# rail-berkeley/serl

Hardware: NVIDIA H100
Metric: drq_critic_grad_steps_per_sec (higher is better)
Workload: dtype f16

## Files before the change

### serl_b200/csrc/stem_pool.cu

```cuda
#include "common.cuh"
#include "conv_common.cuh"
#include "serl_b200.h"
#include "wgmma.cuh"

namespace serl {

constexpr int SP_BOX = 7 * 64 * 32;
constexpr int SP_STAGE = 4 * SP_BOX;
constexpr int SP_STAGES = 3;
constexpr int SP_OFF_A = 4 * 8192;
constexpr int SP_OFF_STG = SP_OFF_A + SP_STAGES * SP_STAGE;
constexpr int SP_OFF_SLOT = SP_OFF_STG + 8 * 1024;
constexpr int SP_OFF_BAR = SP_OFF_SLOT + 4 * 4 * 4 * 2 * 4;
constexpr int SP_SMEM = SP_OFF_BAR + 8 * (2 * SP_STAGES + 5) + 1024;
static_assert((SP_BOX % 1024) == 0 && SP_SMEM <= 232448, "stem_pool_kernel: shared memory layout");

struct StemPoolArgs {
  uint16_t* pooled; uint16_t* side; float* stats; int32_t* error;
  unsigned long long neg_mask; int N;
};

template <class F>
__global__ void __launch_bounds__(CONV_THREADS, 1)
stem_pool_kernel(const __grid_constant__ CUtensorMap xmap, const __grid_constant__ CUtensorMap wmap, const StemPoolArgs a) {
  pdl_prologue();
  extern __shared__ uint8_t smem_raw[];
  uint8_t* smem = reinterpret_cast<uint8_t*>((reinterpret_cast<uintptr_t>(smem_raw) + 1023) & ~(uintptr_t)1023);
  uint8_t* sW = smem;
  uint8_t* sA = smem + SP_OFF_A;
  float* slot = reinterpret_cast<float*>(smem + SP_OFF_SLOT);
  uint64_t* full = reinterpret_cast<uint64_t*>(smem + SP_OFF_BAR);
  uint64_t* empty = full + SP_STAGES;
  uint64_t* wbar = empty + SP_STAGES;
  uint64_t* gnbar = wbar + 1;

  const int warp = threadIdx.x >> 5, lane = threadIdx.x & 31;
  const int band = blockIdx.x & 3;
  const int img0 = blockIdx.x >> 2, img_step = gridDim.x >> 2;

  if (threadIdx.x == 0) {
    for (int s = 0; s < SP_STAGES; ++s) { tc_mbar_init(&full[s], 1); tc_mbar_init(&empty[s], 4); }
    tc_mbar_init(wbar, 1);
    for (int q = 0; q < 4; ++q) tc_mbar_init(&gnbar[q], 1);
    asm volatile("fence.mbarrier_init.release.cluster;" ::: "memory");
  }
  __syncthreads();
  cluster_sync_all();

  if (warp >= 8) {
    asm volatile("setmaxnreg.dec.sync.aligned.u32 40;" ::: "memory");
    if (warp == 8 && lane == 0) {
      asm volatile("prefetch.tensormap [%0];" ::"l"(&xmap) : "memory");
      asm volatile("prefetch.tensormap [%0];" ::"l"(&wmap) : "memory");
      tc_mbar_expect_tx(wbar, 4u * 8192u);
      for (int t = 0; t < 4; ++t) tc_tma_2d(sW + t * 8192, &wmap, t * 64, 0, wbar);
      bool ok = true;
      int pos = 0;
      for (int m = 0; ok; ++m) {
        const int n0 = img0 + 2 * m * img_step;
        if (n0 >= a.N) break;
        const int imgs = n0 + img_step < a.N ? 2 : 1;
        for (int c = 0; c < 4 && ok; ++c)
          for (int g = 0; g < imgs; ++g, ++pos) {
            const int s = pos % SP_STAGES;
            if (!(ok = tc_mbar_wait(&empty[s], ((uint32_t)(pos / SP_STAGES) & 1u) ^ 1u, a.error))) break;
            tc_mbar_expect_tx(&full[s], (uint32_t)SP_STAGE);
            for (int sx = 0; sx < 4; ++sx)
              tc_tma_4d(sA + s * SP_STAGE + sx * SP_BOX, &xmap, 0, sx, 16 * band + 4 * c, n0 + g * img_step, &full[s]);
          }
      }
    }
  } else {
    asm volatile("setmaxnreg.inc.sync.aligned.u32 232;" ::: "memory");
    const int g = warp >> 2, wl = warp & 3, tid = threadIdx.x & 127, quad = lane & 3;
    const uint32_t a_base = smem_u32(sA), w_base = smem_u32(sW);
    const int ch = 16 * wl + (lane >> 2);
    const uint32_t flip = (uint32_t)((a.neg_mask >> ch) & 1ull) * 0x8000u | (uint32_t)((a.neg_mask >> (ch + 8)) & 1ull) * 0x80000000u;
    const int next = (lane & ~3) | ((lane + 1) & 3);
    uint8_t* stg = smem + SP_OFF_STG + warp * 1024;
    const uint32_t mrow = smem_u32(stg) + (uint32_t)(((lane >> 4) * 8 + (lane & 1) * 4 + ((lane >> 1) & 3)) * 32 +
                                                     ((((lane >> 3) ^ lane) & 1) << 4));
    const int gpx = lane >> 1, gh = lane & 1;
    const uint32_t grow = (uint32_t)(gpx * 32 + ((gh ^ (gpx >> 2)) & 1) * 16);
    auto store_row = [&](uint16_t* dst, const uint32_t (&v)[8]) {
      uint32_t o[2][4];
#pragma unroll
      for (int t = 0; t < 4; ++t) {
        o[t >> 1][2 * (t & 1)] = __byte_perm(v[2 * t], v[2 * t + 1], 0x5410);
        o[t >> 1][2 * (t & 1) + 1] = __byte_perm(v[2 * t], v[2 * t + 1], 0x7632);
      }
      stsm_x4_trans(mrow, o[0]);
      stsm_x4_trans(mrow + 512, o[1]);
      __syncwarp();
#pragma unroll
      for (int e = 0; e < 2; ++e)
        *reinterpret_cast<uint4*>(dst + (size_t)(gpx + 16 * e) * 64 + 8 * gh) = *reinterpret_cast<const uint4*>(stg + grow + e * 512);
      __syncwarp();
    };
    bool ok = tc_mbar_wait(wbar, 0u, a.error);
    ok = mma_bar_and(ok);
    auto collect = [&](int m) {
      const int q = 2 * g + (m & 1);
      ok = tc_mbar_wait_cluster(&gnbar[q], (uint32_t)(m >> 1) & 1u, a.error);
      if (ok && band == 0 && lane < 2) {
        float v = 0.f;
#pragma unroll
        for (int rk = 0; rk < 4; ++rk) v += slot[((q * 4 + rk) * 4 + wl) * 2 + lane];
        atomicAdd(a.stats + (size_t)(img0 + (2 * m + g) * img_step) * 8 + wl * 2 + lane, v);
      }
    };
    float acc[128];
    uint32_t carry[8];
    float S = 0.f, SS = 0.f;
    int m = 0;
    for (;; ++m) {
      const int n = img0 + (2 * m + g) * img_step;
      if (n >= a.N) break;
      const bool pair = img0 + (2 * m + 1) * img_step < a.N;
      const bool more = img0 + (2 * m + 2) * img_step < a.N;
      uint16_t* out = a.pooled + (size_t)n * 32 * 2048 + 16 * wl;
      for (int c = 0; c < 4; ++c) {
        const int pos = 8 * m + (pair ? 2 * c + g : c), s = pos % SP_STAGES;
        if (g == 1 || (c > 0 ? pair : m > 0)) named_bar_sync(2 + g, 256);
        if (ok) ok = tc_mbar_wait(&full[s], (uint32_t)(pos / SP_STAGES) & 1u, a.error);
        if (ok) {
          const uint32_t bs = a_base + (uint32_t)(s * SP_STAGE);
          wg_fence();
#pragma unroll
          for (int r = 0; r < 4; ++r)
#pragma unroll
            for (int sx = 0; sx < 4; ++sx)
              wg_mma_h16_n256<F::kBf16>(acc, wg_desc(w_base + (uint32_t)(r * 8192)) + 2 * sx,
                                        wg_desc_sw32(bs + (uint32_t)(sx * SP_BOX + r * 2048)), (uint32_t)(r | sx));
          wg_commit();
        }
        if (g == 0 ? pair : (c < 3 || more)) named_bar_arrive(3 - g, 256);
        wg_wait<0>();
        __syncwarp();
        if (!ok) continue;
        if (lane == 0) tc_mbar_arrive(&empty[s]);

        if (c == 0) {
          if (m > 0) collect(m - 1);
          S = 0.f; SS = 0.f;
        }
#pragma unroll
        for (int j = 0; j < 32; ++j) {
          const float* d = &acc[4 * j];
          S += (d[0] + d[1]) + (d[2] + d[3]);
          SS += (d[0] * d[0] + d[1] * d[1]) + (d[2] * d[2] + d[3] * d[3]);
        }
        uint32_t v[8];
        auto pool_row = [&](int i, bool first) {
          uint32_t w0[8], w1[8];
#pragma unroll
          for (int jj = 0; jj < 8; ++jj) {
            const float* d = &acc[4 * (8 * i + jj)];
            w0[jj] = F::pack(d[0], d[2]) ^ flip;
            w1[jj] = F::pack(d[1], d[3]) ^ flip;
          }
#pragma unroll
          for (int jj = 0; jj < 8; ++jj) {
            const uint32_t nb = __shfl_sync(0xffffffffu, quad == 0 ? w0[jj < 7 ? jj + 1 : 7] : w0[jj], next);
            uint32_t x = first ? w0[jj] : F::max2(v[jj], w0[jj]);
            x = F::max2(x, w1[jj]);
            if (jj < 7 || quad != 3) x = F::max2(x, nb);
            v[jj] = x;
          }
        };
        const int p0 = 8 * band + 2 * c;
        uint32_t o[8];
        pool_row(0, true);
        if (c > 0) {
#pragma unroll
          for (int jj = 0; jj < 8; ++jj) o[jj] = F::max2(carry[jj], v[jj]);
          store_row(out + (size_t)(p0 - 1) * 2048, o);
        } else {
          store_row(a.side + ((size_t)n * 4 + band) * 2048 + 16 * wl, v);
        }
        pool_row(1, false);
#pragma unroll
        for (int jj = 0; jj < 8; ++jj) o[jj] = v[jj];
        pool_row(2, true);
#pragma unroll
        for (int jj = 0; jj < 8; ++jj) o[jj] = F::max2(o[jj], v[jj]);
        store_row(out + (size_t)p0 * 2048, o);
        pool_row(3, false);
        if (c == 3) store_row(out + (size_t)(p0 + 1) * 2048, v);
#pragma unroll
        for (int jj = 0; jj < 8; ++jj) carry[jj] = v[jj];

        if (c == 3) {
          S = warp_sum(S); SS = warp_sum(SS);
          const int q = 2 * g + (m & 1);
          if (tid == 0) tc_mbar_expect_tx(&gnbar[q], 4u * 4u * 2u * 4u);
          if (lane < 2) {
            const float* dst = slot + ((q * 4 + band) * 4 + wl) * 2 + lane;
#pragma unroll
            for (int rk = 0; rk < 4; ++rk) {
              uint32_t rdst, rbar;
              asm volatile("mapa.shared::cluster.u32 %0, %1, %2;" : "=r"(rdst) : "r"(smem_u32(dst)), "r"(rk));
              asm volatile("mapa.shared::cluster.u32 %0, %1, %2;" : "=r"(rbar) : "r"(smem_u32(&gnbar[q])), "r"(rk));
              asm volatile("st.async.shared::cluster.mbarrier::complete_tx::bytes.b32 [%0], %1, [%2];"
                           ::"r"(rdst), "r"(__float_as_uint(lane ? SS : S)), "r"(rbar) : "memory");
            }
          }
        }
      }
    }
    if (ok && m > 0) collect(m - 1);
  }
  cluster_sync_all();
}

template <class F>
static int launch_stem_pool(const serl_stem_pool_desc* d, cudaStream_t st) {
  auto kern = stem_pool_kernel<F>;
  static int clusters = 0;
  if (!clusters) {
    if (cudaFuncSetAttribute(kern, cudaFuncAttributeMaxDynamicSharedMemorySize, SP_SMEM) != cudaSuccess) return check_launch("cudaFuncSetAttribute(stem_pool)");
    int dev = 0, sms = 0, n = 0;
    cudaGetDevice(&dev);
    cudaDeviceGetAttribute(&sms, cudaDevAttrMultiProcessorCount, dev);
    cudaLaunchConfig_t cfg = {};
    cudaLaunchAttribute attr[1];
    attr[0].id = cudaLaunchAttributeClusterDimension;
    attr[0].val.clusterDim.x = 4; attr[0].val.clusterDim.y = 1; attr[0].val.clusterDim.z = 1;
    cfg.gridDim = dim3(4 * sms); cfg.blockDim = dim3(CONV_THREADS); cfg.dynamicSmemBytes = SP_SMEM;
    cfg.attrs = attr; cfg.numAttrs = 1;
    if (cudaOccupancyMaxActiveClusters(&n, kern, &cfg) != cudaSuccess) return check_launch("cudaOccupancyMaxActiveClusters(stem_pool)");
    if (n <= 0) { set_last_error("serl_stem_conv_pool_tc_h16: stem_pool_kernel (%d B shared memory) cannot be resident", SP_SMEM); return SERL_ERR_CUDA; }
    clusters = n;
  }
  TcEncodeTiledFn enc = tc_get_encode();
  if (!enc) { set_last_error("serl_stem_conv_pool_tc_h16: cuTensorMapEncodeTiled unavailable"); return SERL_ERR_CUDA; }
  const CUtensorMapDataType dt = d->fmt == SERL_FMT_FP16 ? CU_TENSOR_MAP_DATA_TYPE_FLOAT16 : CU_TENSOR_MAP_DATA_TYPE_BFLOAT16;
  CUtensorMap xmap, wmap;
  {
    const cuuint64_t gdim[4] = {16u, 67u, 67u, (cuuint64_t)d->N};
    const cuuint64_t gstr[3] = {16u * 2u, 67u * 16u * 2u, 67u * 67u * 16u * 2u};
    const cuuint32_t box[4] = {16u, 64u, 7u, 1u};
    const cuuint32_t estr[4] = {1u, 1u, 1u, 1u};
    CUresult r = enc(&xmap, dt, 4, const_cast<void*>(d->xs), gdim, gstr, box, estr, CU_TENSOR_MAP_INTERLEAVE_NONE, CU_TENSOR_MAP_SWIZZLE_32B,
                     CU_TENSOR_MAP_L2_PROMOTION_L2_256B, CU_TENSOR_MAP_FLOAT_OOB_FILL_NONE);
    if (r != CUDA_SUCCESS) { set_last_error("serl_stem_conv_pool_tc_h16: cuTensorMapEncodeTiled (input) failed (%d)", (int)r); return SERL_ERR_CUDA; }
  }
  {
    const cuuint64_t gdim[2] = {256u, 64u};
    const cuuint64_t gstr[1] = {256u * 2u};
    const cuuint32_t box[2] = {64u, 64u};
    const cuuint32_t estr[2] = {1u, 1u};
    CUresult r = enc(&wmap, dt, 2, const_cast<void*>(d->w), gdim, gstr, box, estr, CU_TENSOR_MAP_INTERLEAVE_NONE, CU_TENSOR_MAP_SWIZZLE_128B,
                     CU_TENSOR_MAP_L2_PROMOTION_L2_256B, CU_TENSOR_MAP_FLOAT_OOB_FILL_NONE);
    if (r != CUDA_SUCCESS) { set_last_error("serl_stem_conv_pool_tc_h16: cuTensorMapEncodeTiled (weights) failed (%d)", (int)r); return SERL_ERR_CUDA; }
  }
  StemPoolArgs a{};
  a.pooled = static_cast<uint16_t*>(d->pooled); a.side = static_cast<uint16_t*>(d->side); a.stats = d->stats; a.error = d->error;
  a.neg_mask = d->neg_mask; a.N = d->N;
  const int rounds = ceil_div(d->N, clusters);
  const int used = ceil_div(d->N, rounds);
  launch_k_cluster(kern, dim3(used * 4), dim3(CONV_THREADS), 4, (size_t)SP_SMEM, st, xmap, wmap, a);
  return check_launch("stem_pool_kernel");
}

}

using namespace serl;

extern "C" int serl_stem_v2_active(void) { return 1; }

extern "C" int serl_stem_conv_pool_tc_h16(const serl_stem_pool_desc* d, void* stream) {
  if (!d || !d->xs || !d->w || !d->pooled || !d->side || !d->stats || !d->error || d->N < 1) {
    set_last_error("serl_stem_conv_pool_tc_h16: invalid descriptor"); return SERL_ERR_INVALID;
  }
  return d->fmt == SERL_FMT_FP16 ? launch_stem_pool<Fp16>(d, static_cast<cudaStream_t>(stream))
                                 : launch_stem_pool<Bf16>(d, static_cast<cudaStream_t>(stream));
}
```

Measured before the change: 522.2.

## Load one input box plus edge strip via TMA and build shifted copies in smem

Instead of issuing four overlapping TMA loads (one per x-shift) for each stage, the producer loads a single 64-wide box plus an 8-wide edge strip. Warps 9-11 and lane 0 of warp 8 then construct the three shifted copies with shared-memory copies and signal the full barrier. This cuts redundant global/L2 traffic by roughly 4x per stage. In exchange it adds a new loaded barrier, extra smem copy work in low-register producer warps, and a proxy fence per stage.

```diff
diff --git a/serl_b200/csrc/stem_pool.cu b/serl_b200/csrc/stem_pool.cu
--- a/serl_b200/csrc/stem_pool.cu
+++ b/serl_b200/csrc/stem_pool.cu
@@ -6,23 +6,36 @@
 namespace serl {
 
 constexpr int SP_BOX = 7 * 64 * 32;
-constexpr int SP_STAGE = 4 * SP_BOX;
+constexpr int SP_EDGE = 7 * 8 * 32;
+constexpr int SP_OFF_EDGE = 4 * SP_BOX;
+constexpr int SP_STAGE = SP_OFF_EDGE + 2048;
 constexpr int SP_STAGES = 3;
 constexpr int SP_OFF_A = 4 * 8192;
 constexpr int SP_OFF_STG = SP_OFF_A + SP_STAGES * SP_STAGE;
 constexpr int SP_OFF_SLOT = SP_OFF_STG + 8 * 1024;
 constexpr int SP_OFF_BAR = SP_OFF_SLOT + 4 * 4 * 4 * 2 * 4;
-constexpr int SP_SMEM = SP_OFF_BAR + 8 * (2 * SP_STAGES + 5) + 1024;
-static_assert((SP_BOX % 1024) == 0 && SP_SMEM <= 232448, "stem_pool_kernel: shared memory layout");
+constexpr int SP_SMEM = SP_OFF_BAR + 8 * (3 * SP_STAGES + 5) + 1024;
+static_assert((SP_BOX % 1024) == 0 && (SP_STAGE % 1024) == 0 && SP_EDGE <= SP_STAGE - SP_OFF_EDGE && SP_SMEM <= 232448,
+              "stem_pool_kernel: shared memory layout");
 
 struct StemPoolArgs {
   uint16_t* pooled; uint16_t* side; float* stats; int32_t* error;
   unsigned long long neg_mask; int N;
 };
 
+__device__ __forceinline__ uint4 lds128(uint32_t addr) {
+  uint4 v;
+  asm volatile("ld.shared.v4.b32 {%0, %1, %2, %3}, [%4];" : "=r"(v.x), "=r"(v.y), "=r"(v.z), "=r"(v.w) : "r"(addr) : "memory");
+  return v;
+}
+__device__ __forceinline__ void sts128(uint32_t addr, const uint4& v) {
+  asm volatile("st.shared.v4.b32 [%0], {%1, %2, %3, %4};" ::"r"(addr), "r"(v.x), "r"(v.y), "r"(v.z), "r"(v.w) : "memory");
+}
+
 template <class F>
 __global__ void __launch_bounds__(CONV_THREADS, 1)
-stem_pool_kernel(const __grid_constant__ CUtensorMap xmap, const __grid_constant__ CUtensorMap wmap, const StemPoolArgs a) {
+stem_pool_kernel(const __grid_constant__ CUtensorMap xmap, const __grid_constant__ CUtensorMap emap,
+                 const __grid_constant__ CUtensorMap wmap, const StemPoolArgs a) {
   pdl_prologue();
   extern __shared__ uint8_t smem_raw[];
   uint8_t* smem = reinterpret_cast<uint8_t*>((reinterpret_cast<uintptr_t>(smem_raw) + 1023) & ~(uintptr_t)1023);
@@ -31,7 +44,8 @@
   float* slot = reinterpret_cast<float*>(smem + SP_OFF_SLOT);
   uint64_t* full = reinterpret_cast<uint64_t*>(smem + SP_OFF_BAR);
   uint64_t* empty = full + SP_STAGES;
-  uint64_t* wbar = empty + SP_STAGES;
+  uint64_t* loaded = empty + SP_STAGES;
+  uint64_t* wbar = loaded + SP_STAGES;
   uint64_t* gnbar = wbar + 1;
 
   const int warp = threadIdx.x >> 5, lane = threadIdx.x & 31;
@@ -39,7 +53,7 @@
   const int img0 = blockIdx.x >> 2, img_step = gridDim.x >> 2;
 
   if (threadIdx.x == 0) {
-    for (int s = 0; s < SP_STAGES; ++s) { tc_mbar_init(&full[s], 1); tc_mbar_init(&empty[s], 4); }
+    for (int s = 0; s < SP_STAGES; ++s) { tc_mbar_init(&full[s], 3); tc_mbar_init(&empty[s], 4); tc_mbar_init(&loaded[s], 1); }
     tc_mbar_init(wbar, 1);
     for (int q = 0; q < 4; ++q) tc_mbar_init(&gnbar[q], 1);
     asm volatile("fence.mbarrier_init.release.cluster;" ::: "memory");
@@ -51,9 +65,18 @@
     asm volatile("setmaxnreg.dec.sync.aligned.u32 40;" ::: "memory");
     if (warp == 8 && lane == 0) {
       asm volatile("prefetch.tensormap [%0];" ::"l"(&xmap) : "memory");
+      asm volatile("prefetch.tensormap [%0];" ::"l"(&emap) : "memory");
       asm volatile("prefetch.tensormap [%0];" ::"l"(&wmap) : "memory");
       tc_mbar_expect_tx(wbar, 4u * 8192u);
       for (int t = 0; t < 4; ++t) tc_tma_2d(sW + t * 8192, &wmap, t * 64, 0, wbar);
+    }
+    if (warp > 8 || lane == 0) {
+      const int sx = warp - 8, xl = lane >> 1, h = lane & 1, xs = xl + sx;
+      const uint32_t src = (uint32_t)(xs * 32 + ((h ^ (xs >> 2)) & 1) * 16);
+      const uint32_t dst = (uint32_t)(sx * SP_BOX + xl * 32 + ((h ^ (xl >> 2)) & 1) * 16);
+      const int e = xs - 16;
+      const uint32_t src3 = e < 0 ? 1536u + src : (uint32_t)(SP_OFF_EDGE + e * 32 + ((h ^ (e >> 2)) & 1) * 16);
+      const uint32_t step3 = e < 0 ? 2048u : 256u;
       bool ok = true;
       int pos = 0;
       for (int m = 0; ok; ++m) {
@@ -63,10 +86,29 @@
         for (int c = 0; c < 4 && ok; ++c)
           for (int g = 0; g < imgs; ++g, ++pos) {
             const int s = pos % SP_STAGES;
-            if (!(ok = tc_mbar_wait(&empty[s], ((uint32_t)(pos / SP_STAGES) & 1u) ^ 1u, a.error))) break;
-            tc_mbar_expect_tx(&full[s], (uint32_t)SP_STAGE);
-            for (int sx = 0; sx < 4; ++sx)
-              tc_tma_4d(sA + s * SP_STAGE + sx * SP_BOX, &xmap, 0, sx, 16 * band + 4 * c, n0 + g * img_step, &full[s]);
+            const uint32_t par = (uint32_t)(pos / SP_STAGES) & 1u;
+            if (warp == 8) {
+              if (!(ok = tc_mbar_wait(&empty[s], par ^ 1u, a.error))) break;
+              tc_mbar_expect_tx(&loaded[s], (uint32_t)(SP_BOX + SP_EDGE));
+              tc_tma_4d(sA + s * SP_STAGE, &xmap, 0, 0, 16 * band + 4 * c, n0 + g * img_step, &loaded[s]);
+              tc_tma_4d(sA + s * SP_STAGE + SP_OFF_EDGE, &emap, 0, 64, 16 * band + 4 * c, n0 + g * img_step, &loaded[s]);
+            } else {
+              ok = __all_sync(0xffffffffu, tc_mbar_wait(&loaded[s], par, a.error));
+              if (!ok) break;
+              const uint32_t st = smem_u32(sA + s * SP_STAGE);
+#pragma unroll
+              for (int y = 0; y < 7; ++y) {
+                uint4 v[4];
+#pragma unroll
+                for (int k = 0; k < 3; ++k) v[k] = lds128(st + src + (uint32_t)(y * 2048 + k * 512));
+                v[3] = lds128(st + src3 + (uint32_t)y * step3);
+#pragma unroll
+                for (int k = 0; k < 4; ++k) sts128(st + dst + (uint32_t)(y * 2048 + k * 512), v[k]);
+              }
+              asm volatile("fence.proxy.async.shared::cta;" ::: "memory");
+              __syncwarp();
+              if (lane == 0) tc_mbar_arrive(&full[s]);
+            }
           }
       }
     }
@@ -235,14 +277,14 @@
   TcEncodeTiledFn enc = tc_get_encode();
   if (!enc) { set_last_error("serl_stem_conv_pool_tc_h16: cuTensorMapEncodeTiled unavailable"); return SERL_ERR_CUDA; }
   const CUtensorMapDataType dt = d->fmt == SERL_FMT_FP16 ? CU_TENSOR_MAP_DATA_TYPE_FLOAT16 : CU_TENSOR_MAP_DATA_TYPE_BFLOAT16;
-  CUtensorMap xmap, wmap;
-  {
+  CUtensorMap xmap, emap, wmap;
+  for (int edge = 0; edge < 2; ++edge) {
     const cuuint64_t gdim[4] = {16u, 67u, 67u, (cuuint64_t)d->N};
     const cuuint64_t gstr[3] = {16u * 2u, 67u * 16u * 2u, 67u * 67u * 16u * 2u};
-    const cuuint32_t box[4] = {16u, 64u, 7u, 1u};
+    const cuuint32_t box[4] = {16u, edge ? 8u : 64u, 7u, 1u};
     const cuuint32_t estr[4] = {1u, 1u, 1u, 1u};
-    CUresult r = enc(&xmap, dt, 4, const_cast<void*>(d->xs), gdim, gstr, box, estr, CU_TENSOR_MAP_INTERLEAVE_NONE, CU_TENSOR_MAP_SWIZZLE_32B,
-                     CU_TENSOR_MAP_L2_PROMOTION_L2_256B, CU_TENSOR_MAP_FLOAT_OOB_FILL_NONE);
+    CUresult r = enc(edge ? &emap : &xmap, dt, 4, const_cast<void*>(d->xs), gdim, gstr, box, estr, CU_TENSOR_MAP_INTERLEAVE_NONE,
+                     CU_TENSOR_MAP_SWIZZLE_32B, CU_TENSOR_MAP_L2_PROMOTION_L2_256B, CU_TENSOR_MAP_FLOAT_OOB_FILL_NONE);
     if (r != CUDA_SUCCESS) { set_last_error("serl_stem_conv_pool_tc_h16: cuTensorMapEncodeTiled (input) failed (%d)", (int)r); return SERL_ERR_CUDA; }
   }
   {
@@ -259,7 +301,7 @@
   a.neg_mask = d->neg_mask; a.N = d->N;
   const int rounds = ceil_div(d->N, clusters);
   const int used = ceil_div(d->N, rounds);
-  launch_k_cluster(kern, dim3(used * 4), dim3(CONV_THREADS), 4, (size_t)SP_SMEM, st, xmap, wmap, a);
+  launch_k_cluster(kern, dim3(used * 4), dim3(CONV_THREADS), 4, (size_t)SP_SMEM, st, xmap, emap, wmap, a);
   return check_launch("stem_pool_kernel");
 }
 
```

Measured after the change: 530.4 (median of 6 runs). +1.6%, better.
